# maturk/dn-splatter

Measured on NVIDIA H100. Metric: rendered Mpix/s (fwd+bwd, RGB+depth+normal), higher is better.
Workload: dtype f32

## Files before the change

dn_splatter_b200/_lib.py:

```python
from __future__ import annotations

import ctypes as C
import os
from typing import Optional

HERE = os.path.dirname(os.path.abspath(__file__))
LIB_PATH = os.path.join(HERE, "libdnr_b200.so")

FLAG_ACTIVATED, FLAG_ANTIALIASED, FLAG_NORMALS, FLAG_ACCUMULATE, FLAG_EXACT_LISTS = 1, 2, 4, 8, 16
FLAG_HOST_CAMERA = 32
FLAG_PERSISTENT_WS = 256
LOSS_FUSED_BWD, LOSS_IMG_U8, LOSS_NORMAL_U8, LOSS_EDGE_FROM_IMAGE = 1, 2, 4, 8
REC_FLOATS, REC_FLOATS_N, GRAD_FLOATS = 12, 16, 16
DEPTH_LOSS_TYPES = {None: 0, "EdgeAwareLogL1": 1, "LogL1": 2, "L1": 3, "MSE": 4}

_f, _i, _p = C.c_float, C.c_int32, C.c_void_p


class DnrArgs(C.Structure):

    _fields_ = [
        ("n_gauss", _i), ("width", _i), ("height", _i), ("tile_size", _i), ("sh_degree", _i), ("sh_bases", _i),
        ("flags", C.c_uint32), ("list_shift", _i),
        ("near_plane", _f), ("far_plane", _f), ("eps2d", _f), ("radius_clip", _f),
# ... 57 lines not shown
class DnrPoissonGrid(C.Structure):

    _fields_ = [("origin", _f * 3), ("cell", _f), ("depth", _i), ("reserved", _i)]


class DnrGridDesc(C.Structure):

    _fields_ = [("origin", _f * 3), ("cell", _f), ("dims", C.c_int32 * 3), ("channels", _i)]


POISSON_MIN_DEPTH, POISSON_MAX_DEPTH, POISSON_MAX_CYCLES = 4, 10, 100
ISO_POSE, ISO_MAX_DEPTH = 36, 10
_d = C.c_double


class DnrIsoFrames(C.Structure):

    _fields_ = [("depth", _p), ("normals", _p), ("poses", _p), ("n_frames", _i), ("width", _i), ("height", _i),
                ("cam_normals", _i), ("K", _d * 9), ("inv_K", _d * 9), ("depth_scale", _d), ("rel_delta", _d)]


class DnrIsoParams(C.Structure):

    _fields_ = [("max_tsdf_rel", _d), ("max_tsdf_abs", _d), ("min_dot", _d), ("use_normals", _i), ("passes", _i)]


class DnrIsoGrid(C.Structure):

    _fields_ = [("origin", _d * 3), ("cell", _d), ("max_depth", _i), ("threshold", _i)]


DN_MAX_K, DN_OMNIDATA, DN_DSINE, DN_DEPTH_TO_NORMAL = 256, 0, 1, 2


class DnrDnPose(C.Structure):

    _fields_ = [("rinv", _d * 9), ("t", _d * 3)]


class DnrDnSearch(C.Structure):

    _fields_ = [("lo", _d * 3), ("cell", _d), ("center", _d * 3), ("k", _i), ("orient", _i)]


POINTER_FIELDS = {n for n, t in DnrArgs._fields_ if t is _p}

_lib: Optional[C.CDLL] = None

KERNELS_PER_CALL = {
    "dnr_project_fwd": (1, 0), "dnr_bin_scan": (2, 8), "dnr_bin_sort": (3, 4), "dnr_raster_fwd": (1, 0),
    "dnr_finalize_fwd": (1, 0), "dnr_normal_from_depth": (1, 0), "dnr_raster_bwd": (1, 0), "dnr_project_bwd": (1, 0),
    "dnr_loss_fwd": (2, 0), "dnr_loss_bwd": (1, 0), "dnr_scale_loss_fwd": (1, 0), "dnr_scale_loss_bwd": (1, 0),
    "dnr_l1_fwd": (1, 0), "dnr_l1_bwd": (1, 0), "dnr_u8_to_f32": (1, 0),
    "dnr_ssim_fwd": (1, 0), "dnr_ssim_bwd": (1, 0), "dnr_ssim_fwd_ex": (1, 0), "dnr_ssim_bwd_ex": (1, 0), "dnr_photometric_fwd": (2, 0), "dnr_photometric_bwd": (1, 0), "dnr_adam_step": (1, 0), "dnr_adam_step_reduce": (2, 0),
    "dnr_grad_zero": (1, 0),
    "dnr_knn_build": (2, 1), "dnr_knn_query": (1, 0), "dnr_density": (1, 0), "dnr_ray_densities": (1, 0),
    "dnr_tsdf_integrate": (1, 0), "dnr_mc_count": (1, 6), "dnr_mc_emit": (2, 0),
    "dnr_grid_sample": (1, 0), "dnr_mesh_visibility": (1, 0),
    "dnr_rgb_metrics": (1, 0), "dnr_depth_metrics": (1, 0), "dnr_normal_metrics": (8, 0),
    "dnr_iso_samples": (2, 2), "dnr_iso_eval": (1, 0), "dnr_iso_corners": (3, 4),
    "dnr_dn_backproject": (1, 0), "dnr_dn_normals": (8, 5), "dnr_dn_consistency": (1, 0),
}
LAUNCHES = {"handwritten": 0, "cub": 0}
DEBUG_CAPTURE = os.environ.get("DNR_DEBUG_CAPTURE") == "1"


def capture_ok(where: str) -> None:
    if not DEBUG_CAPTURE:
        return
    import torch

    try:
        torch.cuda.is_current_stream_capturing()
    except Exception as exc:
        raise DnrError(f"stream capture invalidated by {where}: {exc}") from exc


class _Counting:

    def __init__(self, lib):
        self._lib = lib

    def __getattr__(self, name):
        fn = getattr(self._lib, name)
        k = KERNELS_PER_CALL.get(name)
        if k is None:
            return fn

        def call(*args):
            LAUNCHES["handwritten"] += k[0]
            LAUNCHES["cub"] += k[1]
            rc = fn(*args)
            if DEBUG_CAPTURE:
                capture_ok(f"{name} (rc {rc})")
            return rc

        self.__dict__[name] = call
        return call


class DnrError(RuntimeError):
    pass


def load():
    global _lib
    if _lib is not None:
# ... 189 lines not shown
```

dn_splatter_b200/csrc/ssim.cu:

```cuda
#include "common.cuh"

namespace {

constexpr int SS_R = 5;
constexpr int SS_T = 16;
constexpr int SS_H = SS_T + 2 * SS_R;
constexpr int SS_P = 28;
constexpr int SS_C = 3;
constexpr int SS_NT = 256;

__constant__ float c_win[11] = {1.028380357e-03f, 7.598758209e-03f, 3.600077331e-02f, 1.093606874e-01f, 2.130055279e-01f,
                                2.660117149e-01f, 2.130055279e-01f, 1.093606874e-01f, 3.600077331e-02f, 7.598758209e-03f,
                                1.028380357e-03f};

__device__ __forceinline__ double warp_sum_f64(double v) {
#pragma unroll
  for (int o = 16; o > 0; o >>= 1) v += __shfl_xor_sync(0xffffffffu, v, o);
  return v;
}

template <bool U8>
__device__ __forceinline__ float ld_gt(const void* img, size_t idx) {
  return U8 ? __fmul_rn((float)((const uint8_t*)img)[idx], 1.0f / 255.0f) : ((const float*)img)[idx];
}

template <int NQ_IN, int NQ_OUT, int NC, typename Make>
__device__ __forceinline__ void hpass(float (*s_in)[SS_C][SS_H][SS_P], float (*s_mid)[SS_C][SS_H][SS_T], int tid, Make make) {
  constexpr int items = NC * SS_H * (SS_T / 2);
  for (int it = tid; it < items; it += SS_NT) {
    const int seg = it % (SS_T / 2), r = (it / (SS_T / 2)) % SS_H, c = it / ((SS_T / 2) * SS_H);
    float in[NQ_IN][12];
#pragma unroll
    for (int q = 0; q < NQ_IN; ++q) {
      const float2* p = reinterpret_cast<const float2*>(&s_in[q][c][r][2 * seg]);
#pragma unroll
      for (int k = 0; k < 6; ++k) { const float2 v = p[k]; in[q][2 * k] = v.x; in[q][2 * k + 1] = v.y; }
    }
    float acc[NQ_OUT][2];
#pragma unroll
    for (int q = 0; q < NQ_OUT; ++q) acc[q][0] = acc[q][1] = 0.f;
#pragma unroll
    for (int k = 0; k < 12; ++k) {
      float v[NQ_OUT];
      float src[NQ_IN];
#pragma unroll
      for (int q = 0; q < NQ_IN; ++q) src[q] = in[q][k];
      make(src, v);
#pragma unroll
      for (int q = 0; q < NQ_OUT; ++q) {
        if (k < 11) acc[q][0] += c_win[k] * v[q];
        if (k > 0) acc[q][1] += c_win[k - 1] * v[q];
      }
    }
#pragma unroll
    for (int q = 0; q < NQ_OUT; ++q) *reinterpret_cast<float2*>(&s_mid[q][c][r][2 * seg]) = make_float2(acc[q][0], acc[q][1]);
  }
}

template <int NQ>
__device__ __forceinline__ void vpass(float (*s_mid)[SS_C][SS_H][SS_T], int c, int col, int g, float out[NQ][4]) {
#pragma unroll
  for (int q = 0; q < NQ; ++q) {
    float v[14];
#pragma unroll
    for (int j = 0; j < 14; ++j) v[j] = s_mid[q][c][4 * g + j][col];
#pragma unroll
    for (int o = 0; o < 4; ++o) {
      float acc = 0.f;
#pragma unroll
      for (int k = 0; k < 11; ++k) acc += c_win[k] * v[o + k];
      out[q][o] = acc;
    }
  }
}

template <bool U8, bool L1, int NC, bool METRIC = false>
__global__ void __launch_bounds__(SS_NT) ssim_fwd_kernel(const float* __restrict__ x, const void* __restrict__ y, int H, int W,
                                                        int C, int c0, float* __restrict__ dmaps, float* __restrict__ sum_out) {
  __shared__ __align__(16) float s_in[2][SS_C][SS_H][SS_P];
  __shared__ __align__(16) float s_mid[5][SS_C][SS_H][SS_T];
  __shared__ float red[SS_NT / 32];
  __shared__ float red_l1[SS_NT / 32];
  const int tid = threadIdx.x;
  constexpr int nc = NC;
  const int i0 = blockIdx.y * SS_T - SS_R, j0 = blockIdx.x * SS_T - SS_R;
  if constexpr (METRIC) {
    const size_t img = (size_t)blockIdx.z * H * W * C;
    x += img;
    y = U8 ? (const void*)((const uint8_t*)y + img) : (const void*)((const float*)y + img);
  }
  for (int e = tid; e < SS_H * SS_H * NC; e += SS_NT) {
    const int c = e % NC, q = (e / NC) % SS_H, r = e / (NC * SS_H);
    const int i = i0 + r, j = j0 + q;
    float xv = 0.f, yv = 0.f;
    if (i >= 0 && i < H && j >= 0 && j < W) {
      const size_t p = ((size_t)i * W + j) * C + c0 + c;
      xv = x[p];
      yv = ld_gt<U8>(y, p);
    }
    s_in[0][c][r][q] = xv;
    s_in[1][c][r][q] = yv;
  }
  __syncthreads();
  hpass<2, 5, NC>(s_in, s_mid, tid, [](const float* s, float* v) {
    v[0] = s[0]; v[1] = s[1]; v[2] = s[0] * s[0]; v[3] = s[1] * s[1]; v[4] = s[0] * s[1];
  });
  __syncthreads();
  float ssum = 0.f, lsum = 0.f;
  if (tid < nc * SS_T * 4) {
    const int col = tid % SS_T, g = (tid / SS_T) % 4, c = tid / (SS_T * 4);
    float f[5][4];
    vpass<5>(s_mid, c, col, g, f);
    const int j = blockIdx.x * SS_T + col;
    const size_t n = (size_t)H * W * C;
#pragma unroll
    for (int o = 0; o < 4; ++o) {
      const int i = blockIdx.y * SS_T + 4 * g + o;
      const bool interior = (i >= SS_R) && (i < H - SS_R) && (j >= SS_R) && (j < W - SS_R);
      float s = 0.f, d_mu = 0.f, d_xx = 0.f, d_xy = 0.f;
      if (interior) {
        const float C1 = 0.0001f, C2 = 0.0009f;
        const float mx = f[0][o], my = f[1][o];
        const float sx = f[2][o] - mx * mx, sy = f[3][o] - my * my, sxy = f[4][o] - mx * my;
        const float A1 = 2.f * mx * my + C1, A2 = 2.f * sxy + C2, B1 = mx * mx + my * my + C1, B2 = sx + sy + C2;
        const float inv = 1.0f / (B1 * B2);
        s = A1 * A2 * inv;
        d_xx = -s / B2;
        d_xy = 2.f * A1 * inv;
        d_mu = 2.f * my * (A2 - A1) * inv - 2.f * mx * s / B1 + 2.f * mx * s / B2;
      }
      if (i < H && j < W) {
        const size_t p = ((size_t)i * W + j) * C + c0 + c;
        if constexpr (METRIC) {
          const float d = s_in[0][c][4 * g + o + SS_R][col + SS_R] - s_in[1][c][4 * g + o + SS_R][col + SS_R];
          lsum += d * d;
        } else {
          dmaps[p] = d_mu; dmaps[n + p] = d_xx; dmaps[2 * n + p] = d_xy;
          if (L1) lsum += fabsf(s_in[0][c][4 * g + o + SS_R][col + SS_R] - s_in[1][c][4 * g + o + SS_R][col + SS_R]);
        }
      }
      ssum += s;
    }
  }
  if constexpr (METRIC) {
    __shared__ double red_d[2][SS_NT / 32];
    const double ds = warp_sum_f64(ssum), dl = warp_sum_f64(lsum);
    if ((tid & 31) == 0) { red_d[0][tid >> 5] = ds; red_d[1][tid >> 5] = dl; }
    __syncthreads();
    if (tid == 0) {
      double t = 0.0, tl = 0.0;
#pragma unroll
      for (int w = 0; w < SS_NT / 32; ++w) { t += red_d[0][w]; tl += red_d[1][w]; }
      double* out = reinterpret_cast<double*>(sum_out) + 2 * blockIdx.z;
      if (t != 0.0) atomicAdd(out, t);
      if (tl != 0.0) atomicAdd(out + 1, tl);
    }
    return;
  }
  ssum = warp_sum(ssum);
  if (L1) lsum = warp_sum(lsum);
  if ((tid & 31) == 0) { red[tid >> 5] = ssum; if (L1) red_l1[tid >> 5] = lsum; }
  __syncthreads();
  if (tid == 0) {
    float t = 0.f, tl = 0.f;
#pragma unroll
    for (int w = 0; w < SS_NT / 32; ++w) { t += red[w]; if (L1) tl += red_l1[w]; }
    if (t != 0.f) atomicAdd(sum_out, t);
    if (L1 && tl != 0.f) atomicAdd(sum_out + 1, tl);
  }
}

__global__ void photometric_finish_kernel(float* out, float lambda, float inv_count_ssim, float inv_count_l1) {
  out[2] = (1.0f - lambda) * (out[1] * inv_count_l1) + lambda * (1.0f - out[0] * inv_count_ssim);
}

template <bool U8, int NC>
__global__ void __launch_bounds__(SS_NT) ssim_bwd_kernel(const float* __restrict__ x, const void* __restrict__ y, int H, int W,
                                                        int C, int c0, const float* __restrict__ dmaps, const float* v_mean,
                                                        float w_ssim, float w_l1, float* __restrict__ v_x) {
  __shared__ __align__(16) float s_in[3][SS_C][SS_H][SS_P];
  __shared__ __align__(16) float s_mid[3][SS_C][SS_H][SS_T];
  const int tid = threadIdx.x;
  constexpr int nc = NC;
  const int i0 = blockIdx.y * SS_T - SS_R, j0 = blockIdx.x * SS_T - SS_R;
  const size_t n = (size_t)H * W * C;
  for (int e = tid; e < SS_H * SS_H * NC; e += SS_NT) {
    const int c = e % NC, q = (e / NC) % SS_H, r = e / (NC * SS_H);
    const int i = i0 + r, j = j0 + q;
    float a = 0.f, b = 0.f, d = 0.f;
    if (i >= 0 && i < H && j >= 0 && j < W) {
      const size_t p = ((size_t)i * W + j) * C + c0 + c;
      a = dmaps[p]; b = dmaps[n + p]; d = dmaps[2 * n + p];
    }
    s_in[0][c][r][q] = a; s_in[1][c][r][q] = b; s_in[2][c][r][q] = d;
  }
  __syncthreads();
  hpass<3, 3, NC>(s_in, s_mid, tid, [](const float* s, float* v) { v[0] = s[0]; v[1] = s[1]; v[2] = s[2]; });
  __syncthreads();
  if (tid < nc * SS_T * 4) {
    const int col = tid % SS_T, g = (tid / SS_T) % 4, c = tid / (SS_T * 4);
    float f[3][4];
    vpass<3>(s_mid, c, col, g, f);
    const int j = blockIdx.x * SS_T + col;
    const float count = (float)(H - 2 * SS_R) * (float)(W - 2 * SS_R) * (float)C;
    const float vm = v_mean ? __ldg(v_mean) : 1.0f;
    const float gsc = vm * w_ssim / count;
    const float gl1 = vm * w_l1 / ((float)H * (float)W * (float)C);
#pragma unroll
    for (int o = 0; o < 4; ++o) {
      const int i = blockIdx.y * SS_T + 4 * g + o;
      if (i < H && j < W) {
        const size_t p = ((size_t)i * W + j) * C + c0 + c;
        const float xv = x[p], yv = ld_gt<U8>(y, p);
        const float d = xv - yv;
        v_x[p] = gsc * (f[0][o] + 2.f * xv * f[1][o] + yv * f[2][o]) + gl1 * ((d > 0.f) ? 1.f : ((d < 0.f) ? -1.f : 0.f));
      }
    }
  }
}

}

template <bool L1>
static int launch_ssim_fwd(const float* pred, const void* gt, int gt_is_u8, int H, int W, int C, float* dmaps, float* out, cudaStream_t s) {
  const dim3 grid((W + SS_T - 1) / SS_T, (H + SS_T - 1) / SS_T, 1);
  for (int c0 = 0; c0 < C; c0 += SS_C) {
    const int nc = C - c0 < SS_C ? C - c0 : SS_C;
#define DNR_SSIM_FWD(U8, NC) ssim_fwd_kernel<U8, L1, NC><<<grid, SS_NT, 0, s>>>(pred, gt, H, W, C, c0, dmaps, out)
    if (gt_is_u8) { if (nc == 3) DNR_SSIM_FWD(true, 3); else if (nc == 2) DNR_SSIM_FWD(true, 2); else DNR_SSIM_FWD(true, 1); }
    else { if (nc == 3) DNR_SSIM_FWD(false, 3); else if (nc == 2) DNR_SSIM_FWD(false, 2); else DNR_SSIM_FWD(false, 1); }
#undef DNR_SSIM_FWD
    DNR_CHECK_LAUNCH();
  }
  return 0;
}

static int launch_ssim_bwd(const float* pred, const void* gt, int gt_is_u8, int H, int W, int C, const float* dmaps, const float* v,
                           float w_ssim, float w_l1, float* v_pred, cudaStream_t s) {
  const dim3 grid((W + SS_T - 1) / SS_T, (H + SS_T - 1) / SS_T, 1);
  for (int c0 = 0; c0 < C; c0 += SS_C) {
    const int nc = C - c0 < SS_C ? C - c0 : SS_C;
#define DNR_SSIM_BWD(U8, NC) ssim_bwd_kernel<U8, NC><<<grid, SS_NT, 0, s>>>(pred, gt, H, W, C, c0, dmaps, v, w_ssim, w_l1, v_pred)
    if (gt_is_u8) { if (nc == 3) DNR_SSIM_BWD(true, 3); else if (nc == 2) DNR_SSIM_BWD(true, 2); else DNR_SSIM_BWD(true, 1); }
    else { if (nc == 3) DNR_SSIM_BWD(false, 3); else if (nc == 2) DNR_SSIM_BWD(false, 2); else DNR_SSIM_BWD(false, 1); }
#undef DNR_SSIM_BWD
    DNR_CHECK_LAUNCH();
  }
  return 0;
}

extern "C" int dnr_rgb_metrics(const float* pred, const void* gt, int32_t gt_is_u8, int32_t B, int32_t H, int32_t W, int32_t C,
                               double* out, void* stream) {
  if (!pred || !gt || !out) return DNR_E_NULL;
  if (B <= 0 || B > 65535 || H <= 2 * SS_R || W <= 2 * SS_R || C <= 0) return DNR_E_SIZE;
  cudaStream_t s = (cudaStream_t)stream;
  DNR_CUDA(cudaMemsetAsync(out, 0, 2 * (size_t)B * sizeof(double), s));
  const dim3 grid((W + SS_T - 1) / SS_T, (H + SS_T - 1) / SS_T, B);
  float* o = reinterpret_cast<float*>(out);
  for (int c0 = 0; c0 < C; c0 += SS_C) {
    const int nc = C - c0 < SS_C ? C - c0 : SS_C;
#define DNR_SSIM_MET(U8, NC) ssim_fwd_kernel<U8, false, NC, true><<<grid, SS_NT, 0, s>>>(pred, gt, H, W, C, c0, nullptr, o)
    if (gt_is_u8) { if (nc == 3) DNR_SSIM_MET(true, 3); else if (nc == 2) DNR_SSIM_MET(true, 2); else DNR_SSIM_MET(true, 1); }
    else { if (nc == 3) DNR_SSIM_MET(false, 3); else if (nc == 2) DNR_SSIM_MET(false, 2); else DNR_SSIM_MET(false, 1); }
#undef DNR_SSIM_MET
    DNR_CHECK_LAUNCH();
  }
  return 0;
}

extern "C" int dnr_ssim_fwd_ex(const float* pred, const void* gt, int32_t gt_is_u8, int32_t H, int32_t W, int32_t C, float* dmaps,
                               float* sum_out, void* stream) {
  if (!pred || !gt || !dmaps || !sum_out) return DNR_E_NULL;
  if (H <= 2 * SS_R || W <= 2 * SS_R || C <= 0) return DNR_E_SIZE;
  cudaStream_t s = (cudaStream_t)stream;
  DNR_CUDA(cudaMemsetAsync(sum_out, 0, sizeof(float), s));
  return launch_ssim_fwd<false>(pred, gt, gt_is_u8, H, W, C, dmaps, sum_out, s);
}

extern "C" int dnr_photometric_fwd(const float* pred, const void* gt, int32_t gt_is_u8, int32_t H, int32_t W, int32_t C,
                                   float ssim_lambda, float* dmaps, float* out, void* stream) {
  if (!pred || !gt || !dmaps || !out) return DNR_E_NULL;
  if (H <= 2 * SS_R || W <= 2 * SS_R || C <= 0) return DNR_E_SIZE;
  cudaStream_t s = (cudaStream_t)stream;
  DNR_CUDA(cudaMemsetAsync(out, 0, 3 * sizeof(float), s));
  if (const int rc = launch_ssim_fwd<true>(pred, gt, gt_is_u8, H, W, C, dmaps, out, s)) return rc;
  photometric_finish_kernel<<<1, 1, 0, s>>>(out, ssim_lambda, 1.0f / ((float)(H - 2 * SS_R) * (float)(W - 2 * SS_R) * (float)C),
                                            1.0f / ((float)H * (float)W * (float)C));
  DNR_CHECK_LAUNCH();
  return 0;
}

extern "C" int dnr_photometric_bwd(const float* pred, const void* gt, int32_t gt_is_u8, int32_t H, int32_t W, int32_t C,
                                   float ssim_lambda, const float* dmaps, const float* v_main, float* v_pred, void* stream) {
  if (!pred || !gt || !dmaps || !v_pred) return DNR_E_NULL;
  if (H <= 2 * SS_R || W <= 2 * SS_R || C <= 0) return DNR_E_SIZE;
  return launch_ssim_bwd(pred, gt, gt_is_u8, H, W, C, dmaps, v_main, -ssim_lambda, 1.0f - ssim_lambda, v_pred, (cudaStream_t)stream);
}

extern "C" int dnr_ssim_bwd_ex(const float* pred, const void* gt, int32_t gt_is_u8, int32_t H, int32_t W, int32_t C,
                               const float* dmaps, const float* v_mean, float* v_pred, void* stream) {
  if (!pred || !gt || !dmaps || !v_pred) return DNR_E_NULL;
  if (H <= 2 * SS_R || W <= 2 * SS_R || C <= 0) return DNR_E_SIZE;
  return launch_ssim_bwd(pred, gt, gt_is_u8, H, W, C, dmaps, v_mean, 1.0f, 0.0f, v_pred, (cudaStream_t)stream);
}

extern "C" int dnr_ssim_fwd(const float* pred, const float* gt, int32_t H, int32_t W, int32_t C, float* dmaps, float* sum_out,
                            void* stream) {
  return dnr_ssim_fwd_ex(pred, gt, 0, H, W, C, dmaps, sum_out, stream);
}

extern "C" int dnr_ssim_bwd(const float* pred, const float* gt, int32_t H, int32_t W, int32_t C, const float* dmaps,
                            const float* v_mean, float* v_pred, void* stream) {
  return dnr_ssim_bwd_ex(pred, gt, 0, H, W, C, dmaps, v_mean, v_pred, stream);
}
```

dn_splatter_b200/regularization_strategy.py:

```python
from __future__ import annotations

import ctypes as C
from abc import abstractmethod
from typing import Optional

import torch
import torch.nn as nn
import torch.nn.functional as F
from torch import Tensor

from . import _lib as L
from .losses import DepthLoss, DepthLossType, NormalLoss, NormalLossType

_FUSED_DEPTH = {DepthLossType.EdgeAwareLogL1: 1, DepthLossType.LogL1: 2, DepthLossType.L1: 3, DepthLossType.MSE: 4}


def _shared_holder(*tensors):
    from .rasterize import raster_holder

    hs = [raster_holder(t) for t in tensors if t is not None]
    if not hs or any(h is None for h in hs) or any(h is not hs[0] for h in hs):
        return None
    return hs[0]


class _FusedDNLoss(torch.autograd.Function):

    @staticmethod
    def forward(ctx, pred_depth, pred_normal, gt_depth, gt_normal, gt_img, depth_type: int, depth_lambda: float,
                depth_tolerance: float, use_normal: bool, holder=None, edge_image=None):
        lib = L.load()
        ref = pred_depth if pred_depth is not None else pred_normal
        if ref.device.type != "cuda":
            raise L.DnrError("DNRegularization: the fused regulariser needs CUDA tensors (no CPU path)")
        if depth_type:
            H, W = pred_depth.shape[0], pred_depth.shape[1]
        else:
            H, W = pred_normal.shape[0], pred_normal.shape[1]
        dev = ref.device

        def prep(t, keep_u8=False):
            if t is None:
                return None
            if keep_u8 and t.dtype == torch.uint8:
                return t.detach().to(device=dev).contiguous()
            return t.detach().to(device=dev, dtype=torch.float32).contiguous()

        pd, pn, gd, gi = prep(pred_depth), prep(pred_normal), prep(gt_depth), prep(gt_img)
        gn = prep(gt_normal, keep_u8=True)
        ei = prep(edge_image, keep_u8=True)
        flags = 0
        if gn is not None and gn.dtype == torch.uint8:
            flags |= L.LOSS_NORMAL_U8
        if ei is not None:
            assert ei.dtype == torch.uint8, "edge_image is the raw uint8 image"
            flags |= L.LOSS_EDGE_FROM_IMAGE | L.LOSS_IMG_U8
        partials = torch.empty(12, dtype=torch.float32, device=dev)
        a = L.DnrArgs()
        a.width, a.height = W, H
        a.depth_loss_type, a.use_normal_loss = int(depth_type), int(bool(use_normal))
        a.depth_lambda, a.depth_tolerance = float(depth_lambda), float(depth_tolerance)
        a.loss_flags = flags
        for k, t in dict(out_depth=pd, out_normal=pn, gt_depth=gd, gt_normal=gn, gt_rgb=gi, gt_image=ei,
                         loss_partials=partials).items():
            setattr(a, k, None if t is None else t.data_ptr())
        L.check(lib.dnr_loss_fwd(C.byref(a), L.stream()), "dnr_loss_fwd")
        ctx.keep = (pd, pn, gd, gn, gi, ei, partials)
        ctx.fwd_stream = torch.cuda.current_stream()
        ctx.cfg = (W, H, int(depth_type), int(bool(use_normal)), float(depth_lambda), float(depth_tolerance), flags)
        ctx.shapes = (None if pred_depth is None else pred_depth.shape, None if pred_normal is None else pred_normal.shape)
        ctx.holder = holder
        return partials[11].clone()

    @staticmethod
    def backward(ctx, v):
        with torch.cuda.stream(ctx.fwd_stream):
            return _FusedDNLoss._backward(ctx, v)

    @staticmethod
    def _backward(ctx, v):
        lib = L.load()
        pd, pn, gd, gn, gi, ei, partials = ctx.keep
        W, H, depth_type, use_normal, lam, tol, flags = ctx.cfg
        v = v.detach().to(torch.float32).contiguous()
        none9 = (None,) * 9
        if ctx.holder is not None:
            from .rasterize import zero_token

            ctx.holder.setdefault("deferred", {})["reg"] = dict(
                depth_type=depth_type, use_normal=use_normal, depth_lambda=lam, depth_tolerance=tol, gt_depth=gd,
                gt_normal=gn if use_normal else None, gt_rgb=gi, edge_image=ei, loss_partials=partials, v=v)
            vd = zero_token(pd.view(ctx.shapes[0])) if (depth_type and ctx.needs_input_grad[0]) else None
            vn = zero_token(pn.view(ctx.shapes[1])) if (use_normal and ctx.needs_input_grad[1]) else None
            return (vd, vn) + none9
        a = L.DnrArgs()
        a.width, a.height = W, H
        a.depth_loss_type, a.use_normal_loss, a.depth_lambda, a.depth_tolerance = depth_type, use_normal, lam, tol
        a.loss_flags = flags
        for k, t in dict(out_depth=pd, out_normal=pn, gt_depth=gd, gt_normal=gn, gt_rgb=gi, gt_image=ei,
                         loss_partials=partials, v_loss=v).items():
            setattr(a, k, None if t is None else t.data_ptr())
        vd = torch.empty(ctx.shapes[0], dtype=torch.float32, device=v.device) if (depth_type and ctx.needs_input_grad[0]) else None
        vn = torch.empty(ctx.shapes[1], dtype=torch.float32, device=v.device) if (use_normal and ctx.needs_input_grad[1]) else None
        if vd is not None or vn is not None:
            L.check(lib.dnr_loss_bwd(C.byref(a), None if vd is None else vd.data_ptr(),
                                     None if vn is None else vn.data_ptr(), L.stream()), "dnr_loss_bwd")
        return (vd, vn) + none9


class _ScaleLoss(torch.autograd.Function):

    @staticmethod
    def forward(ctx, scales):
        lib = L.load()
        if scales.device.type != "cuda":
            raise L.DnrError("scale loss: CUDA tensor required (no CPU path)")
        s = scales.detach().float().contiguous()
        out = torch.empty(1, dtype=torch.float32, device=s.device)
        L.check(lib.dnr_scale_loss_fwd(s.data_ptr(), s.shape[0], out.data_ptr(), L.stream()), "dnr_scale_loss_fwd")
        ctx.s = s
        ctx.fwd_stream = torch.cuda.current_stream()
        return out[0].clone()

    @staticmethod
    def backward(ctx, v):
        with torch.cuda.stream(ctx.fwd_stream):
            return _ScaleLoss._backward(ctx, v)

    @staticmethod
    def _backward(ctx, v):
        lib = L.load()
        s = ctx.s
        v = v.detach().float().contiguous()
        g = torch.empty_like(s)
        L.check(lib.dnr_scale_loss_bwd(s.data_ptr(), s.shape[0], v.data_ptr(), g.data_ptr(), L.stream()),
                "dnr_scale_loss_bwd")
        return g


class FusedL1(torch.autograd.Function):

    @staticmethod
    def forward(ctx, pred, gt, holder=None):
        lib = L.load()
        if pred.device.type != "cuda" or gt.device != pred.device:
            raise L.DnrError("FusedL1 needs CUDA tensors on one device (no CPU path)")
        p = pred.detach().float().contiguous()
        g = gt.detach().contiguous()
        if g.dtype != torch.uint8:
            g = g.float()
        assert g.numel() == p.numel(), "pred / gt size mismatch"
        out = torch.empty(1, dtype=torch.float32, device=p.device)
        L.check(lib.dnr_l1_fwd(p.data_ptr(), g.data_ptr(), p.numel(), int(g.dtype == torch.uint8), out.data_ptr(), L.stream()),
                "dnr_l1_fwd")
        ctx.keep = (p, g)
        ctx.shape = pred.shape
        ctx.fwd_stream = torch.cuda.current_stream()
        ctx.holder = holder
        return out[0].clone()

    @staticmethod
    def backward(ctx, v):
        with torch.cuda.stream(ctx.fwd_stream):
            return FusedL1._backward(ctx, v)

    @staticmethod
    def _backward(ctx, v):
        lib = L.load()
        p, g = ctx.keep
        v = v.detach().float().contiguous()
        if ctx.holder is not None:
            from .rasterize import zero_token

            ctx.holder.setdefault("deferred", {})["l1"] = dict(gt=g, v=v)
            return zero_token(p.view(ctx.shape)), None, None
        vp = torch.empty_like(p)
        L.check(lib.dnr_l1_bwd(p.data_ptr(), g.data_ptr(), p.numel(), int(g.dtype == torch.uint8), v.data_ptr(), vp.data_ptr(),
                               L.stream()), "dnr_l1_bwd")
        return vp.view(ctx.shape), None, None


class FusedSSIM(torch.autograd.Function):

    @staticmethod
    def forward(ctx, pred, gt):
        lib = L.load()
        if pred.device.type != "cuda" or gt.device != pred.device:
            raise L.DnrError("FusedSSIM needs CUDA tensors on one device (no CPU path)")
        p = pred.detach().float().contiguous()
        g = gt.detach().contiguous()
        if g.dtype != torch.uint8:
            g = g.float()
        assert p.dim() == 3 and p.shape == g.shape, "pred / gt must both be [H,W,C]"
        H, W, Cn = p.shape
        dmaps = torch.empty((3, H, W, Cn), dtype=torch.float32, device=p.device)
        out = torch.empty(1, dtype=torch.float32, device=p.device)
        L.check(lib.dnr_ssim_fwd_ex(p.data_ptr(), g.data_ptr(), int(g.dtype == torch.uint8), H, W, Cn, dmaps.data_ptr(),
                                    out.data_ptr(), L.stream()), "dnr_ssim_fwd_ex")
        ctx.keep = (p, g, dmaps)
        ctx.fwd_stream = torch.cuda.current_stream()
        return out[0] / float((H - 10) * (W - 10) * Cn)

    @staticmethod
    def backward(ctx, v):
        with torch.cuda.stream(ctx.fwd_stream):
            lib = L.load()
            p, g, dmaps = ctx.keep
            v = v.detach().float().contiguous()
            vp = torch.empty_like(p)
            H, W, Cn = p.shape
            L.check(lib.dnr_ssim_bwd_ex(p.data_ptr(), g.data_ptr(), int(g.dtype == torch.uint8), H, W, Cn, dmaps.data_ptr(),
                                        v.data_ptr(), vp.data_ptr(), L.stream()), "dnr_ssim_bwd_ex")
            return vp, None


class FusedPhotometric(torch.autograd.Function):

    @staticmethod
    def forward(ctx, pred, gt, ssim_lambda: float):
        lib = L.load()
        if pred.device.type != "cuda" or gt.device != pred.device:
            raise L.DnrError("FusedPhotometric needs CUDA tensors on one device (no CPU path)")
        p = pred.detach().float().contiguous()
        g = gt.detach().contiguous()
        if g.dtype != torch.uint8:
            g = g.float()
        assert p.dim() == 3 and p.shape == g.shape, "pred / gt must both be [H,W,C]"
        H, W, Cn = p.shape
        dmaps = torch.empty((3, H, W, Cn), dtype=torch.float32, device=p.device)
        out = torch.empty(3, dtype=torch.float32, device=p.device)
        L.check(lib.dnr_photometric_fwd(p.data_ptr(), g.data_ptr(), int(g.dtype == torch.uint8), H, W, Cn, float(ssim_lambda),
                                        dmaps.data_ptr(), out.data_ptr(), L.stream()), "dnr_photometric_fwd")
        ctx.keep = (p, g, dmaps)
        ctx.lam = float(ssim_lambda)
        ctx.fwd_stream = torch.cuda.current_stream()
        return out[2].clone()

    @staticmethod
    def backward(ctx, v):
        with torch.cuda.stream(ctx.fwd_stream):
            lib = L.load()
            p, g, dmaps = ctx.keep
            v = v.detach().float().contiguous()
            vp = torch.empty_like(p)
            H, W, Cn = p.shape
            L.check(lib.dnr_photometric_bwd(p.data_ptr(), g.data_ptr(), int(g.dtype == torch.uint8), H, W, Cn, ctx.lam,
                                            dmaps.data_ptr(), v.data_ptr(), vp.data_ptr(), L.stream()), "dnr_photometric_bwd")
            return vp, None, None


def u8_to_float(img: Tensor, divisor: float = 255.0, clamp_min: float = 0.0) -> Tensor:
    src = img.contiguous()
    dst = torch.empty(src.shape, dtype=torch.float32, device=src.device)
    L.check(L.load().dnr_u8_to_f32(src.data_ptr(), src.numel(), float(divisor), float(clamp_min), dst.data_ptr(), L.stream()),
            "dnr_u8_to_f32")
    return dst


class RegularizationStrategy(nn.Module):

    def __init__(self, **kwargs):
        super().__init__()
        self.device_indicator_param = nn.Parameter(torch.empty(0))

    @property
    def device(self):
        return self.device_indicator_param.device

    @abstractmethod
    def get_loss(self, **kwargs):
        """Loss"""

    def forward(self, **kwargs):
        return self.get_loss(**kwargs)

    def get_scale_loss(self, scales):
        return _ScaleLoss.apply(scales)


class DNRegularization(RegularizationStrategy):

    def __init__(self, depth_tolerance: float = 0.1,
                 depth_loss_type: Optional[DepthLossType] = DepthLossType.EdgeAwareLogL1,
                 depth_lambda: float = 0.2, normal_lambda: float = 0.1):
        super().__init__()
        self.depth_tolerance = depth_tolerance
        self.depth_loss_type = depth_loss_type
        self.depth_loss = DepthLoss(self.depth_loss_type)
        self.depth_lambda = depth_lambda
        self.normal_loss_type = NormalLossType.L1
        self.normal_loss = NormalLoss(self.normal_loss_type)
        self.normal_smooth_loss_type = NormalLossType.Smooth
        self.normal_smooth_loss = NormalLoss(self.normal_smooth_loss_type)
        self.normal_lambda = normal_lambda

    def _fusable(self, with_depth: bool) -> bool:
        return (not with_depth) or self.depth_loss_type in _FUSED_DEPTH

    fuse_backward = True
    """Hand the backward of the fused terms to dnr_raster_bwd when the maps are direct raster outputs; DNSplatterModel sets
# ... 110 lines not shown
```

Before: 781.3.

## Retile SSIM kernels to 32x16, cut shared memory, fuse photometric finish

```diff
diff --git a/dn_splatter_b200/_lib.py b/dn_splatter_b200/_lib.py
--- a/dn_splatter_b200/_lib.py
+++ b/dn_splatter_b200/_lib.py
@@ -133,7 +133,7 @@
     "dnr_finalize_fwd": (1, 0), "dnr_normal_from_depth": (1, 0), "dnr_raster_bwd": (1, 0), "dnr_project_bwd": (1, 0),
     "dnr_loss_fwd": (2, 0), "dnr_loss_bwd": (1, 0), "dnr_scale_loss_fwd": (1, 0), "dnr_scale_loss_bwd": (1, 0),
     "dnr_l1_fwd": (1, 0), "dnr_l1_bwd": (1, 0), "dnr_u8_to_f32": (1, 0),
-    "dnr_ssim_fwd": (1, 0), "dnr_ssim_bwd": (1, 0), "dnr_ssim_fwd_ex": (1, 0), "dnr_ssim_bwd_ex": (1, 0), "dnr_photometric_fwd": (2, 0), "dnr_photometric_bwd": (1, 0), "dnr_adam_step": (1, 0), "dnr_adam_step_reduce": (2, 0),
+    "dnr_ssim_fwd": (1, 0), "dnr_ssim_bwd": (1, 0), "dnr_ssim_fwd_ex": (1, 0), "dnr_ssim_bwd_ex": (1, 0), "dnr_photometric_fwd": (1, 0), "dnr_photometric_bwd": (1, 0), "dnr_adam_step": (1, 0), "dnr_adam_step_reduce": (2, 0),
     "dnr_grad_zero": (1, 0),
     "dnr_knn_build": (2, 1), "dnr_knn_query": (1, 0), "dnr_density": (1, 0), "dnr_ray_densities": (1, 0),
     "dnr_tsdf_integrate": (1, 0), "dnr_mc_count": (1, 6), "dnr_mc_emit": (2, 0),
diff --git a/dn_splatter_b200/csrc/ssim.cu b/dn_splatter_b200/csrc/ssim.cu
--- a/dn_splatter_b200/csrc/ssim.cu
+++ b/dn_splatter_b200/csrc/ssim.cu
@@ -3,11 +3,14 @@
 namespace {
 
 constexpr int SS_R = 5;
-constexpr int SS_T = 16;
-constexpr int SS_H = SS_T + 2 * SS_R;
-constexpr int SS_P = 28;
+constexpr int SS_TW = 32;
+constexpr int SS_TH = 16;
+constexpr int SS_HW = SS_TW + 2 * SS_R;
+constexpr int SS_HH = SS_TH + 2 * SS_R;
+constexpr int SS_P = 44;
 constexpr int SS_C = 3;
 constexpr int SS_NT = 256;
+static_assert(SS_NT == SS_TW * (SS_TH / 2), "one thread per (column, row pair) of the output tile");
 
 __constant__ float c_win[11] = {1.028380357e-03f, 7.598758209e-03f, 3.600077331e-02f, 1.093606874e-01f, 2.130055279e-01f,
                                 2.660117149e-01f, 2.130055279e-01f, 1.093606874e-01f, 3.600077331e-02f, 7.598758209e-03f,
@@ -24,104 +27,145 @@
   return U8 ? __fmul_rn((float)((const uint8_t*)img)[idx], 1.0f / 255.0f) : ((const float*)img)[idx];
 }
 
-template <int NQ_IN, int NQ_OUT, int NC, typename Make>
-__device__ __forceinline__ void hpass(float (*s_in)[SS_C][SS_H][SS_P], float (*s_mid)[SS_C][SS_H][SS_T], int tid, Make make) {
-  constexpr int items = NC * SS_H * (SS_T / 2);
-  for (int it = tid; it < items; it += SS_NT) {
-    const int seg = it % (SS_T / 2), r = (it / (SS_T / 2)) % SS_H, c = it / ((SS_T / 2) * SS_H);
-    float in[NQ_IN][12];
-#pragma unroll
-    for (int q = 0; q < NQ_IN; ++q) {
-      const float2* p = reinterpret_cast<const float2*>(&s_in[q][c][r][2 * seg]);
-#pragma unroll
-      for (int k = 0; k < 6; ++k) { const float2 v = p[k]; in[q][2 * k] = v.x; in[q][2 * k + 1] = v.y; }
-    }
+using HaloPlane = float[SS_C][SS_HH][SS_P];
+using MidPlane = float[SS_C][SS_HH][SS_TW];
+
+template <int NQ_IN, int NQ_OUT, typename Make>
+__device__ __forceinline__ void hitem(const HaloPlane* s_in, int c, int r, int seg, Make make, float acc[NQ_OUT][2]) {
+  float in[NQ_IN][12];
+#pragma unroll
+  for (int q = 0; q < NQ_IN; ++q) {
+    const float2* p = reinterpret_cast<const float2*>(&s_in[q][c][r][2 * seg]);
+#pragma unroll
+    for (int k = 0; k < 6; ++k) { const float2 v = p[k]; in[q][2 * k] = v.x; in[q][2 * k + 1] = v.y; }
+  }
+#pragma unroll
+  for (int q = 0; q < NQ_OUT; ++q) acc[q][0] = acc[q][1] = 0.f;
+#pragma unroll
+  for (int k = 0; k < 12; ++k) {
+    float v[NQ_OUT];
+    float src[NQ_IN];
+#pragma unroll
+    for (int q = 0; q < NQ_IN; ++q) src[q] = in[q][k];
+    make(src, v);
+#pragma unroll
+    for (int q = 0; q < NQ_OUT; ++q) {
+      if (k < 11) acc[q][0] += c_win[k] * v[q];
+      if (k > 0) acc[q][1] += c_win[k - 1] * v[q];
+    }
+  }
+}
+
+constexpr int hpass_items(int nc) { return nc * SS_HH * (SS_TW / 2); }
+
+template <int NQ, int NC, int BATCH, typename Load>
+__device__ __forceinline__ void load_halo(HaloPlane* s_in, int tid, int i0, int j0, int H, int W, int C, int c0, Load load) {
+  constexpr int n = SS_HH * SS_HW * NC, iters = (n + SS_NT - 1) / SS_NT;
+#pragma unroll
+  for (int k0 = 0; k0 < iters; k0 += BATCH) {
+    float v[BATCH][NQ];
+    int off[BATCH];
+#pragma unroll
+    for (int k = 0; k < BATCH; ++k) {
+      const int e = tid + (k0 + k) * SS_NT;
+      off[k] = -1;
+#pragma unroll
+      for (int q = 0; q < NQ; ++q) v[k][q] = 0.f;
+      if (k0 + k < iters && e < n) {
+        const int c = e % NC, q = (e / NC) % SS_HW, r = e / (NC * SS_HW);
+        const int i = i0 + r, j = j0 + q;
+        off[k] = (c * SS_HH + r) * SS_P + q;
+        if (i >= 0 && i < H && j >= 0 && j < W) load(((size_t)i * W + j) * C + c0 + c, v[k]);
+      }
+    }
+#pragma unroll
+    for (int k = 0; k < BATCH; ++k) {
+      if (off[k] >= 0) {
+#pragma unroll
+        for (int q = 0; q < NQ; ++q) (&s_in[q][0][0][0])[off[k]] = v[k][q];
+      }
+    }
+  }
+}
+
+template <int NQ_OUT, int NC, typename Make>
+__device__ __forceinline__ void hpass(const HaloPlane* s_in, MidPlane* s_mid, int tid, Make make) {
+  for (int it = tid; it < hpass_items(NC); it += SS_NT) {
+    const int seg = it % (SS_TW / 2), r = (it / (SS_TW / 2)) % SS_HH, c = it / ((SS_TW / 2) * SS_HH);
     float acc[NQ_OUT][2];
-#pragma unroll
-    for (int q = 0; q < NQ_OUT; ++q) acc[q][0] = acc[q][1] = 0.f;
-#pragma unroll
-    for (int k = 0; k < 12; ++k) {
-      float v[NQ_OUT];
-      float src[NQ_IN];
-#pragma unroll
-      for (int q = 0; q < NQ_IN; ++q) src[q] = in[q][k];
-      make(src, v);
-#pragma unroll
-      for (int q = 0; q < NQ_OUT; ++q) {
-        if (k < 11) acc[q][0] += c_win[k] * v[q];
-        if (k > 0) acc[q][1] += c_win[k - 1] * v[q];
-      }
-    }
+    hitem<2, NQ_OUT>(s_in, c, r, seg, make, acc);
 #pragma unroll
     for (int q = 0; q < NQ_OUT; ++q) *reinterpret_cast<float2*>(&s_mid[q][c][r][2 * seg]) = make_float2(acc[q][0], acc[q][1]);
   }
 }
 
-template <int NQ>
-__device__ __forceinline__ void vpass(float (*s_mid)[SS_C][SS_H][SS_T], int c, int col, int g, float out[NQ][4]) {
+template <int NQ, int NC>
+__device__ __forceinline__ void vpass(const MidPlane* s_mid, int col, int g, float out[NQ][NC][2]) {
 #pragma unroll
   for (int q = 0; q < NQ; ++q) {
-    float v[14];
-#pragma unroll
-    for (int j = 0; j < 14; ++j) v[j] = s_mid[q][c][4 * g + j][col];
-#pragma unroll
-    for (int o = 0; o < 4; ++o) {
-      float acc = 0.f;
-#pragma unroll
-      for (int k = 0; k < 11; ++k) acc += c_win[k] * v[o + k];
-      out[q][o] = acc;
+#pragma unroll
+    for (int c = 0; c < NC; ++c) {
+      float v[12];
+#pragma unroll
+      for (int j = 0; j < 12; ++j) v[j] = s_mid[q][c][2 * g + j][col];
+#pragma unroll
+      for (int o = 0; o < 2; ++o) {
+        float acc = 0.f;
+#pragma unroll
+        for (int k = 0; k < 11; ++k) acc += c_win[k] * v[o + k];
+        out[q][c][o] = acc;
+      }
     }
   }
 }
 
 template <bool U8, bool L1, int NC, bool METRIC = false>
 __global__ void __launch_bounds__(SS_NT) ssim_fwd_kernel(const float* __restrict__ x, const void* __restrict__ y, int H, int W,
-                                                        int C, int c0, float* __restrict__ dmaps, float* __restrict__ sum_out) {
-  __shared__ __align__(16) float s_in[2][SS_C][SS_H][SS_P];
-  __shared__ __align__(16) float s_mid[5][SS_C][SS_H][SS_T];
+                                                        int C, int c0, float* __restrict__ dmaps, float* __restrict__ sum_out,
+                                                        int finish, float lambda, float inv_count_ssim, float inv_count_l1) {
+  __shared__ __align__(16) HaloPlane s_in[2];
+  __shared__ __align__(16) MidPlane s_mid[2];
   __shared__ float red[SS_NT / 32];
   __shared__ float red_l1[SS_NT / 32];
   const int tid = threadIdx.x;
-  constexpr int nc = NC;
-  const int i0 = blockIdx.y * SS_T - SS_R, j0 = blockIdx.x * SS_T - SS_R;
+  const int i0 = blockIdx.y * SS_TH - SS_R, j0 = blockIdx.x * SS_TW - SS_R;
   if constexpr (METRIC) {
     const size_t img = (size_t)blockIdx.z * H * W * C;
     x += img;
     y = U8 ? (const void*)((const uint8_t*)y + img) : (const void*)((const float*)y + img);
   }
-  for (int e = tid; e < SS_H * SS_H * NC; e += SS_NT) {
-    const int c = e % NC, q = (e / NC) % SS_H, r = e / (NC * SS_H);
-    const int i = i0 + r, j = j0 + q;
-    float xv = 0.f, yv = 0.f;
-    if (i >= 0 && i < H && j >= 0 && j < W) {
-      const size_t p = ((size_t)i * W + j) * C + c0 + c;
-      xv = x[p];
-      yv = ld_gt<U8>(y, p);
-    }
-    s_in[0][c][r][q] = xv;
-    s_in[1][c][r][q] = yv;
-  }
-  __syncthreads();
-  hpass<2, 5, NC>(s_in, s_mid, tid, [](const float* s, float* v) {
-    v[0] = s[0]; v[1] = s[1]; v[2] = s[0] * s[0]; v[3] = s[1] * s[1]; v[4] = s[0] * s[1];
+  load_halo<2, NC, (SS_HH * SS_HW * NC + SS_NT - 1) / SS_NT>(s_in, tid, i0, j0, H, W, C, c0, [&](size_t p, float* v) {
+    v[0] = x[p];
+    v[1] = ld_gt<U8>(y, p);
   });
   __syncthreads();
+  const int col = tid % SS_TW, g = tid / SS_TW;
+  float fx[2][NC][2], fy[2][NC][2], fxy[1][NC][2];
+  hpass<2, NC>(s_in, s_mid, tid, [](const float* s, float* v) { v[0] = s[0]; v[1] = s[0] * s[0]; });
+  __syncthreads();
+  vpass<2, NC>(s_mid, col, g, fx);
+  __syncthreads();
+  hpass<2, NC>(s_in, s_mid, tid, [](const float* s, float* v) { v[0] = s[1]; v[1] = s[1] * s[1]; });
+  __syncthreads();
+  vpass<2, NC>(s_mid, col, g, fy);
+  __syncthreads();
+  hpass<1, NC>(s_in, s_mid, tid, [](const float* s, float* v) { v[0] = s[0] * s[1]; });
+  __syncthreads();
+  vpass<1, NC>(s_mid, col, g, fxy);
   float ssum = 0.f, lsum = 0.f;
-  if (tid < nc * SS_T * 4) {
-    const int col = tid % SS_T, g = (tid / SS_T) % 4, c = tid / (SS_T * 4);
-    float f[5][4];
-    vpass<5>(s_mid, c, col, g, f);
-    const int j = blockIdx.x * SS_T + col;
-    const size_t n = (size_t)H * W * C;
-#pragma unroll
-    for (int o = 0; o < 4; ++o) {
-      const int i = blockIdx.y * SS_T + 4 * g + o;
+  const int j = blockIdx.x * SS_TW + col;
+  const size_t n = (size_t)H * W * C;
+#pragma unroll
+  for (int c = 0; c < NC; ++c) {
+#pragma unroll
+    for (int o = 0; o < 2; ++o) {
+      const int i = blockIdx.y * SS_TH + 2 * g + o;
       const bool interior = (i >= SS_R) && (i < H - SS_R) && (j >= SS_R) && (j < W - SS_R);
       float s = 0.f, d_mu = 0.f, d_xx = 0.f, d_xy = 0.f;
       if (interior) {
         const float C1 = 0.0001f, C2 = 0.0009f;
-        const float mx = f[0][o], my = f[1][o];
-        const float sx = f[2][o] - mx * mx, sy = f[3][o] - my * my, sxy = f[4][o] - mx * my;
+        const float mx = fx[0][c][o], my = fy[0][c][o];
+        const float sx = fx[1][c][o] - mx * mx, sy = fy[1][c][o] - my * my, sxy = fxy[0][c][o] - mx * my;
         const float A1 = 2.f * mx * my + C1, A2 = 2.f * sxy + C2, B1 = mx * mx + my * my + C1, B2 = sx + sy + C2;
         const float inv = 1.0f / (B1 * B2);
         s = A1 * A2 * inv;
@@ -132,11 +176,11 @@
       if (i < H && j < W) {
         const size_t p = ((size_t)i * W + j) * C + c0 + c;
         if constexpr (METRIC) {
-          const float d = s_in[0][c][4 * g + o + SS_R][col + SS_R] - s_in[1][c][4 * g + o + SS_R][col + SS_R];
+          const float d = s_in[0][c][2 * g + o + SS_R][col + SS_R] - s_in[1][c][2 * g + o + SS_R][col + SS_R];
           lsum += d * d;
         } else {
           dmaps[p] = d_mu; dmaps[n + p] = d_xx; dmaps[2 * n + p] = d_xy;
-          if (L1) lsum += fabsf(s_in[0][c][4 * g + o + SS_R][col + SS_R] - s_in[1][c][4 * g + o + SS_R][col + SS_R]);
+          if (L1) lsum += fabsf(s_in[0][c][2 * g + o + SS_R][col + SS_R] - s_in[1][c][2 * g + o + SS_R][col + SS_R]);
         }
       }
       ssum += s;
@@ -167,66 +211,93 @@
     for (int w = 0; w < SS_NT / 32; ++w) { t += red[w]; if (L1) tl += red_l1[w]; }
     if (t != 0.f) atomicAdd(sum_out, t);
     if (L1 && tl != 0.f) atomicAdd(sum_out + 1, tl);
-  }
-}
-
-__global__ void photometric_finish_kernel(float* out, float lambda, float inv_count_ssim, float inv_count_l1) {
-  out[2] = (1.0f - lambda) * (out[1] * inv_count_l1) + lambda * (1.0f - out[0] * inv_count_ssim);
+    if constexpr (L1) {
+      if (finish) {
+        __threadfence();
+        const unsigned ticket = atomicAdd(reinterpret_cast<unsigned*>(sum_out + 2), 1u);
+        if (ticket == gridDim.x * gridDim.y - 1) {
+          __threadfence();
+          const float s0 = __ldcg(sum_out), s1 = __ldcg(sum_out + 1);
+          sum_out[2] = (1.0f - lambda) * (s1 * inv_count_l1) + lambda * (1.0f - s0 * inv_count_ssim);
+        }
+      }
+    }
+  }
 }
 
 template <bool U8, int NC>
 __global__ void __launch_bounds__(SS_NT) ssim_bwd_kernel(const float* __restrict__ x, const void* __restrict__ y, int H, int W,
                                                         int C, int c0, const float* __restrict__ dmaps, const float* v_mean,
                                                         float w_ssim, float w_l1, float* __restrict__ v_x) {
-  __shared__ __align__(16) float s_in[3][SS_C][SS_H][SS_P];
-  __shared__ __align__(16) float s_mid[3][SS_C][SS_H][SS_T];
+  __shared__ __align__(16) HaloPlane s_in[3];
   const int tid = threadIdx.x;
-  constexpr int nc = NC;
-  const int i0 = blockIdx.y * SS_T - SS_R, j0 = blockIdx.x * SS_T - SS_R;
+  const int i0 = blockIdx.y * SS_TH - SS_R, j0 = blockIdx.x * SS_TW - SS_R;
   const size_t n = (size_t)H * W * C;
-  for (int e = tid; e < SS_H * SS_H * NC; e += SS_NT) {
-    const int c = e % NC, q = (e / NC) % SS_H, r = e / (NC * SS_H);
-    const int i = i0 + r, j = j0 + q;
-    float a = 0.f, b = 0.f, d = 0.f;
-    if (i >= 0 && i < H && j >= 0 && j < W) {
-      const size_t p = ((size_t)i * W + j) * C + c0 + c;
-      a = dmaps[p]; b = dmaps[n + p]; d = dmaps[2 * n + p];
-    }
-    s_in[0][c][r][q] = a; s_in[1][c][r][q] = b; s_in[2][c][r][q] = d;
-  }
-  __syncthreads();
-  hpass<3, 3, NC>(s_in, s_mid, tid, [](const float* s, float* v) { v[0] = s[0]; v[1] = s[1]; v[2] = s[2]; });
-  __syncthreads();
-  if (tid < nc * SS_T * 4) {
-    const int col = tid % SS_T, g = (tid / SS_T) % 4, c = tid / (SS_T * 4);
-    float f[3][4];
-    vpass<3>(s_mid, c, col, g, f);
-    const int j = blockIdx.x * SS_T + col;
-    const float count = (float)(H - 2 * SS_R) * (float)(W - 2 * SS_R) * (float)C;
-    const float vm = v_mean ? __ldg(v_mean) : 1.0f;
-    const float gsc = vm * w_ssim / count;
-    const float gl1 = vm * w_l1 / ((float)H * (float)W * (float)C);
-#pragma unroll
-    for (int o = 0; o < 4; ++o) {
-      const int i = blockIdx.y * SS_T + 4 * g + o;
+  load_halo<3, NC, 7>(s_in, tid, i0, j0, H, W, C, c0, [&](size_t p, float* v) {
+    v[0] = dmaps[p]; v[1] = dmaps[n + p]; v[2] = dmaps[2 * n + p];
+  });
+  __syncthreads();
+  const int col = tid % SS_TW, g = tid / SS_TW;
+  float f[3][NC][2];
+  constexpr int ipt = (hpass_items(NC) + SS_NT - 1) / SS_NT;
+#pragma unroll
+  for (int q = 0; q < 3; ++q) {
+    float h[ipt][1][2];
+#pragma unroll
+    for (int k = 0; k < ipt; ++k) {
+      const int it = tid + k * SS_NT;
+      if (it < hpass_items(NC))
+        hitem<1, 1>(s_in + q, it / ((SS_TW / 2) * SS_HH), (it / (SS_TW / 2)) % SS_HH, it % (SS_TW / 2),
+                    [](const float* s, float* v) { v[0] = s[0]; }, h[k]);
+    }
+    __syncthreads();
+    MidPlane* mid = reinterpret_cast<MidPlane*>(&s_in[q][0][0][0]);
+#pragma unroll
+    for (int k = 0; k < ipt; ++k) {
+      const int it = tid + k * SS_NT;
+      if (it < hpass_items(NC)) {
+        const int seg = it % (SS_TW / 2), r = (it / (SS_TW / 2)) % SS_HH, c = it / ((SS_TW / 2) * SS_HH);
+        *reinterpret_cast<float2*>(&mid[0][c][r][2 * seg]) = make_float2(h[k][0][0], h[k][0][1]);
+      }
+    }
+    __syncthreads();
+    vpass<1, NC>(mid, col, g, &f[q]);
+  }
+  const int j = blockIdx.x * SS_TW + col;
+  const float count = (float)(H - 2 * SS_R) * (float)(W - 2 * SS_R) * (float)C;
+  const float vm = v_mean ? __ldg(v_mean) : 1.0f;
+  const float gsc = vm * w_ssim / count;
+  const float gl1 = vm * w_l1 / ((float)H * (float)W * (float)C);
+#pragma unroll
+  for (int c = 0; c < NC; ++c) {
+#pragma unroll
+    for (int o = 0; o < 2; ++o) {
+      const int i = blockIdx.y * SS_TH + 2 * g + o;
       if (i < H && j < W) {
         const size_t p = ((size_t)i * W + j) * C + c0 + c;
         const float xv = x[p], yv = ld_gt<U8>(y, p);
         const float d = xv - yv;
-        v_x[p] = gsc * (f[0][o] + 2.f * xv * f[1][o] + yv * f[2][o]) + gl1 * ((d > 0.f) ? 1.f : ((d < 0.f) ? -1.f : 0.f));
-      }
-    }
-  }
-}
-
-}
+        v_x[p] = gsc * (f[0][c][o] + 2.f * xv * f[1][c][o] + yv * f[2][c][o]) + gl1 * ((d > 0.f) ? 1.f : ((d < 0.f) ? -1.f : 0.f));
+      }
+    }
+  }
+}
+
+}
+
+static dim3 ssim_grid(int H, int W, int B) { return dim3((W + SS_TW - 1) / SS_TW, (H + SS_TH - 1) / SS_TH, B); }
 
 template <bool L1>
-static int launch_ssim_fwd(const float* pred, const void* gt, int gt_is_u8, int H, int W, int C, float* dmaps, float* out, cudaStream_t s) {
-  const dim3 grid((W + SS_T - 1) / SS_T, (H + SS_T - 1) / SS_T, 1);
+static int launch_ssim_fwd(const float* pred, const void* gt, int gt_is_u8, int H, int W, int C, float* dmaps, float* out,
+                           float lambda, cudaStream_t s) {
+  const dim3 grid = ssim_grid(H, W, 1);
+  const float inv_ssim = 1.0f / ((float)(H - 2 * SS_R) * (float)(W - 2 * SS_R) * (float)C);
+  const float inv_l1 = 1.0f / ((float)H * (float)W * (float)C);
   for (int c0 = 0; c0 < C; c0 += SS_C) {
     const int nc = C - c0 < SS_C ? C - c0 : SS_C;
-#define DNR_SSIM_FWD(U8, NC) ssim_fwd_kernel<U8, L1, NC><<<grid, SS_NT, 0, s>>>(pred, gt, H, W, C, c0, dmaps, out)
+    const int finish = L1 && c0 + nc == C;
+#define DNR_SSIM_FWD(U8, NC) \
+  ssim_fwd_kernel<U8, L1, NC><<<grid, SS_NT, 0, s>>>(pred, gt, H, W, C, c0, dmaps, out, finish, lambda, inv_ssim, inv_l1)
     if (gt_is_u8) { if (nc == 3) DNR_SSIM_FWD(true, 3); else if (nc == 2) DNR_SSIM_FWD(true, 2); else DNR_SSIM_FWD(true, 1); }
     else { if (nc == 3) DNR_SSIM_FWD(false, 3); else if (nc == 2) DNR_SSIM_FWD(false, 2); else DNR_SSIM_FWD(false, 1); }
 #undef DNR_SSIM_FWD
@@ -237,7 +308,7 @@
 
 static int launch_ssim_bwd(const float* pred, const void* gt, int gt_is_u8, int H, int W, int C, const float* dmaps, const float* v,
                            float w_ssim, float w_l1, float* v_pred, cudaStream_t s) {
-  const dim3 grid((W + SS_T - 1) / SS_T, (H + SS_T - 1) / SS_T, 1);
+  const dim3 grid = ssim_grid(H, W, 1);
   for (int c0 = 0; c0 < C; c0 += SS_C) {
     const int nc = C - c0 < SS_C ? C - c0 : SS_C;
 #define DNR_SSIM_BWD(U8, NC) ssim_bwd_kernel<U8, NC><<<grid, SS_NT, 0, s>>>(pred, gt, H, W, C, c0, dmaps, v, w_ssim, w_l1, v_pred)
@@ -255,11 +326,11 @@
   if (B <= 0 || B > 65535 || H <= 2 * SS_R || W <= 2 * SS_R || C <= 0) return DNR_E_SIZE;
   cudaStream_t s = (cudaStream_t)stream;
   DNR_CUDA(cudaMemsetAsync(out, 0, 2 * (size_t)B * sizeof(double), s));
-  const dim3 grid((W + SS_T - 1) / SS_T, (H + SS_T - 1) / SS_T, B);
+  const dim3 grid = ssim_grid(H, W, B);
   float* o = reinterpret_cast<float*>(out);
   for (int c0 = 0; c0 < C; c0 += SS_C) {
     const int nc = C - c0 < SS_C ? C - c0 : SS_C;
-#define DNR_SSIM_MET(U8, NC) ssim_fwd_kernel<U8, false, NC, true><<<grid, SS_NT, 0, s>>>(pred, gt, H, W, C, c0, nullptr, o)
+#define DNR_SSIM_MET(U8, NC) ssim_fwd_kernel<U8, false, NC, true><<<grid, SS_NT, 0, s>>>(pred, gt, H, W, C, c0, nullptr, o, 0, 0.f, 0.f, 0.f)
     if (gt_is_u8) { if (nc == 3) DNR_SSIM_MET(true, 3); else if (nc == 2) DNR_SSIM_MET(true, 2); else DNR_SSIM_MET(true, 1); }
     else { if (nc == 3) DNR_SSIM_MET(false, 3); else if (nc == 2) DNR_SSIM_MET(false, 2); else DNR_SSIM_MET(false, 1); }
 #undef DNR_SSIM_MET
@@ -274,7 +345,7 @@
   if (H <= 2 * SS_R || W <= 2 * SS_R || C <= 0) return DNR_E_SIZE;
   cudaStream_t s = (cudaStream_t)stream;
   DNR_CUDA(cudaMemsetAsync(sum_out, 0, sizeof(float), s));
-  return launch_ssim_fwd<false>(pred, gt, gt_is_u8, H, W, C, dmaps, sum_out, s);
+  return launch_ssim_fwd<false>(pred, gt, gt_is_u8, H, W, C, dmaps, sum_out, 0.f, s);
 }
 
 extern "C" int dnr_photometric_fwd(const float* pred, const void* gt, int32_t gt_is_u8, int32_t H, int32_t W, int32_t C,
@@ -283,11 +354,7 @@
   if (H <= 2 * SS_R || W <= 2 * SS_R || C <= 0) return DNR_E_SIZE;
   cudaStream_t s = (cudaStream_t)stream;
   DNR_CUDA(cudaMemsetAsync(out, 0, 3 * sizeof(float), s));
-  if (const int rc = launch_ssim_fwd<true>(pred, gt, gt_is_u8, H, W, C, dmaps, out, s)) return rc;
-  photometric_finish_kernel<<<1, 1, 0, s>>>(out, ssim_lambda, 1.0f / ((float)(H - 2 * SS_R) * (float)(W - 2 * SS_R) * (float)C),
-                                            1.0f / ((float)H * (float)W * (float)C));
-  DNR_CHECK_LAUNCH();
-  return 0;
+  return launch_ssim_fwd<true>(pred, gt, gt_is_u8, H, W, C, dmaps, out, ssim_lambda, s);
 }
 
 extern "C" int dnr_photometric_bwd(const float* pred, const void* gt, int32_t gt_is_u8, int32_t H, int32_t W, int32_t C,
diff --git a/dn_splatter_b200/regularization_strategy.py b/dn_splatter_b200/regularization_strategy.py
--- a/dn_splatter_b200/regularization_strategy.py
+++ b/dn_splatter_b200/regularization_strategy.py
@@ -11,6 +11,7 @@
 
 from . import _lib as L
 from .losses import DepthLoss, DepthLossType, NormalLoss, NormalLossType
+from .rasterize import _timed
 
 _FUSED_DEPTH = {DepthLossType.EdgeAwareLogL1: 1, DepthLossType.LogL1: 2, DepthLossType.L1: 3, DepthLossType.MSE: 4}
 
@@ -64,7 +65,7 @@
         for k, t in dict(out_depth=pd, out_normal=pn, gt_depth=gd, gt_normal=gn, gt_rgb=gi, gt_image=ei,
                          loss_partials=partials).items():
             setattr(a, k, None if t is None else t.data_ptr())
-        L.check(lib.dnr_loss_fwd(C.byref(a), L.stream()), "dnr_loss_fwd")
+        L.check(_timed("loss_fwd", lib.dnr_loss_fwd, C.byref(a), L.stream()), "dnr_loss_fwd")
         ctx.keep = (pd, pn, gd, gn, gi, ei, partials)
         ctx.fwd_stream = torch.cuda.current_stream()
         ctx.cfg = (W, H, int(depth_type), int(bool(use_normal)), float(depth_lambda), float(depth_tolerance), flags)
@@ -117,7 +118,8 @@
             raise L.DnrError("scale loss: CUDA tensor required (no CPU path)")
         s = scales.detach().float().contiguous()
         out = torch.empty(1, dtype=torch.float32, device=s.device)
-        L.check(lib.dnr_scale_loss_fwd(s.data_ptr(), s.shape[0], out.data_ptr(), L.stream()), "dnr_scale_loss_fwd")
+        L.check(_timed("scale_loss", lib.dnr_scale_loss_fwd, s.data_ptr(), s.shape[0], out.data_ptr(), L.stream()),
+                "dnr_scale_loss_fwd")
         ctx.s = s
         ctx.fwd_stream = torch.cuda.current_stream()
         return out[0].clone()
@@ -133,7 +135,7 @@
         s = ctx.s
         v = v.detach().float().contiguous()
         g = torch.empty_like(s)
-        L.check(lib.dnr_scale_loss_bwd(s.data_ptr(), s.shape[0], v.data_ptr(), g.data_ptr(), L.stream()),
+        L.check(_timed("scale_loss", lib.dnr_scale_loss_bwd, s.data_ptr(), s.shape[0], v.data_ptr(), g.data_ptr(), L.stream()),
                 "dnr_scale_loss_bwd")
         return g
 
@@ -229,8 +231,8 @@
         H, W, Cn = p.shape
         dmaps = torch.empty((3, H, W, Cn), dtype=torch.float32, device=p.device)
         out = torch.empty(3, dtype=torch.float32, device=p.device)
-        L.check(lib.dnr_photometric_fwd(p.data_ptr(), g.data_ptr(), int(g.dtype == torch.uint8), H, W, Cn, float(ssim_lambda),
-                                        dmaps.data_ptr(), out.data_ptr(), L.stream()), "dnr_photometric_fwd")
+        L.check(_timed("photometric_fwd", lib.dnr_photometric_fwd, p.data_ptr(), g.data_ptr(), int(g.dtype == torch.uint8), H,
+                       W, Cn, float(ssim_lambda), dmaps.data_ptr(), out.data_ptr(), L.stream()), "dnr_photometric_fwd")
         ctx.keep = (p, g, dmaps)
         ctx.lam = float(ssim_lambda)
         ctx.fwd_stream = torch.cuda.current_stream()
@@ -244,8 +246,9 @@
             v = v.detach().float().contiguous()
             vp = torch.empty_like(p)
             H, W, Cn = p.shape
-            L.check(lib.dnr_photometric_bwd(p.data_ptr(), g.data_ptr(), int(g.dtype == torch.uint8), H, W, Cn, ctx.lam,
-                                            dmaps.data_ptr(), v.data_ptr(), vp.data_ptr(), L.stream()), "dnr_photometric_bwd")
+            L.check(_timed("photometric_bwd", lib.dnr_photometric_bwd, p.data_ptr(), g.data_ptr(), int(g.dtype == torch.uint8),
+                           H, W, Cn, ctx.lam, dmaps.data_ptr(), v.data_ptr(), vp.data_ptr(), L.stream()),
+                    "dnr_photometric_bwd")
             return vp, None, None
 
 
```

Result: faster. 794.7, median of 6 (+1.7%).
